# mnlevy1981/MOM6

Measured on AMD Instinct MI355X. Metric: simulated-years/day (SYPD) of the split-RK2 dynamical core + tracer advection + ALE remap, higher is better.
Workload: dtype f64

## Files before the change

### include/mom6hip.h

```cpp
#ifndef MOM6HIP_H
#define MOM6HIP_H

#include <stdint.h>

#ifdef __cplusplus
extern "C" {
#endif

#define MOM6HIP_MEM_HOST   0
#define MOM6HIP_MEM_DEVICE 1

#define MOM6HIP_ADV_PLM    0
#define MOM6HIP_ADV_PPM_H3 1
#define MOM6HIP_ADV_PPM    2

typedef struct mom6hip_grid {
  int32_t isc, iec, jsc, jec;
  int32_t isd, ied, jsd, jed;
  int32_t nk;
  int32_t symmetric;
  int32_t reentrant_x, reentrant_y;
  int32_t first_direction;
  int32_t tripolar_n;
  double Angstrom_H;
// ... 331 lines not shown
                           const mom6hip_bt_cont_t *BT_cont, double *du_cor, double *dv_cor, int32_t memspace);


#define MOM6HIP_EOS_LINEAR 1
#define MOM6HIP_EOS_UNESCO 2
#define MOM6HIP_EOS_WRIGHT 3
#define MOM6HIP_EOS_WRIGHT_FULL 4
#define MOM6HIP_EOS_WRIGHT_REDUCED 5

typedef struct mom6hip_eos {
  int32_t form;
  int32_t reserved;
  double Rho_T0_S0, dRho_dT, dRho_dS;
} mom6hip_eos_t;

typedef struct mom6hip_pressureforce_cs {
  double Rho0;
  double GFS_scale;
  double Z_ref;
  int32_t reconstruct;
  int32_t Recon_Scheme;
  int32_t boundary_extrap;
  int32_t useMassWghtInterp;
  int32_t use_ALE;
  int32_t nkmb;
  double P_Ref;
  const double *Rlay;
  const double *g_prime;
} mom6hip_pressureforce_cs_t;

int mom6hip_pressureforce_fv_bouss(mom6hip_ctx_t *ctx, const mom6hip_pressureforce_cs_t *cs, const mom6hip_eos_t *eos,
                                   const double *h, const double *T, const double *S, const double *p_atm,
                                   double *PFu, double *PFv, double *pbce, double *eta, int32_t memspace);

int mom6hip_pressureforce_fv_nonbouss(mom6hip_ctx_t *ctx, const mom6hip_pressureforce_cs_t *cs, const mom6hip_eos_t *eos,
                                      const double *h, const double *T, const double *S, const double *p_atm, double H_to_RZ,
                                      double *PFu, double *PFv, double *pbce, double *eta, int32_t memspace);

int mom6hip_calculate_density(mom6hip_ctx_t *ctx, const mom6hip_eos_t *eos, const double *T, const double *S,
                              const double *pressure, double *rho, int64_t n, int32_t use_rho_ref, double rho_ref,
                              int32_t memspace);


#define MOM6HIP_BT_HARMONIC     1
#define MOM6HIP_BT_ARITHMETIC   2
#define MOM6HIP_BT_HYBRID       3
#define MOM6HIP_BT_FROM_BT_CONT 4

typedef struct mom6hip_barotropic_cs {
  double dtbt;
  double dtbt_max;
  double dtbt_fraction;
  double bebt;
  double dt_bt_filter;
  double vel_underflow;
  double G_extra;
  double BT_Coriolis_scale;
  double Z_ref;
  double maxCFL_BT_cont;
  double reserved0[6];
  int32_t Sadourny;
  int32_t linearized_BT_PV;
  int32_t strong_drag;
  int32_t visc_rem_u_uh0;
  int32_t adjust_BT_cont;
  int32_t use_wide_halos;
// ... 416 lines not shown
```

### mom6_amd/_lib.py

```python
import ctypes as C
import os

from . import _abi

_HERE = os.path.dirname(os.path.abspath(__file__))
LIB_PATH = os.environ.get("MOM6HIP_LIB_PATH") or os.path.join(_HERE, "libmom6hip.so")
_LIB = None
_dp = C.POINTER(C.c_double)

EXPORTS = (
    "mom6hip_init", "mom6hip_last_error", "mom6hip_grid_create", "mom6hip_grid_destroy",
    "mom6hip_sync", "mom6hip_malloc", "mom6hip_free", "mom6hip_sync_to_device",
    "mom6hip_sync_to_host", "mom6hip_halo_update", "mom6hip_advect_tracer", "mom6hip_set_timing",
    "mom6hip_advect_get_timing", "mom6hip_ale_remap_tracers", "mom6hip_ale_plm_edge_values", "mom6hip_coradcalc", "mom6hip_continuity", "mom6hip_pressureforce_fv_bouss", "mom6hip_pressureforce_fv_nonbouss", "mom6hip_calculate_density", "mom6hip_set_domain_callbacks",
    "mom6hip_barotropic_init", "mom6hip_btcalc", "mom6hip_bt_mass_source", "mom6hip_set_dtbt", "mom6hip_memset_zero", "mom6hip_transfer_stats", "mom6hip_debug_poison_passes", "mom6hip_tracer_hordiff_varmix", "mom6hip_tracer_hordiff_neutral", "mom6hip_tracer_hordiff_epipycnal", "mom6hip_continuity_obc", "mom6hip_coradcalc_obc", "mom6hip_vertvisc_coef_obc", "mom6hip_update_segment_tracer_reservoirs", "mom6hip_advect_tracer_obc", "mom6hip_btstep_obc", "mom6hip_horizontal_viscosity_obc", "mom6hip_set_viscous_bbl_obc", "mom6hip_btcalc_obc", "mom6hip_vertvisc_obc", "mom6hip_radiation_open_bdry_conds", "mom6hip_open_boundary_zero_normal_flow", "mom6hip_overlap_stats", "mom6hip_thickness_diffuse", "mom6hip_mixedlayer_restrat", "mom6hip_mixedlayer_restrat_mu", "mom6hip_start_group_pass", "mom6hip_complete_group_pass", "mom6hip_set_dtbt_eta", "mom6hip_btstep",
    "mom6hip_dyn_split_rk2_init", "mom6hip_step_dyn_split_rk2", "mom6hip_dyn_split_rk2b_init", "mom6hip_step_dyn_split_rk2b",
    "mom6hip_ale_regrid", "mom6hip_ale_remap_set_h_vel", "mom6hip_ale_remap_set_h_vel_via_dz", "mom6hip_ale_remap_velocities", "mom6hip_halo_pack", "mom6hip_set_min_callback", "mom6hip_kernel_timing", "mom6hip_set_callback_stream_ordered", "mom6hip_bt_graph_stats", "mom6hip_bt_graph_nodes",
    "mom6hip_vertvisc_coef", "mom6hip_vertvisc", "mom6hip_vertvisc_remnant", "mom6hip_vertvisc_ntrunc", "mom6hip_vertvisc_and_remnant", "mom6hip_vertvisc_step",
    "mom6hip_hor_visc_init", "mom6hip_horizontal_viscosity", "mom6hip_set_viscous_bbl", "mom6hip_set_viscous_ml",
    "mom6hip_chksum", "mom6hip_reproducing_sum", "mom6hip_write_energy_sums", "mom6hip_depth_list_create", "mom6hip_write_energy_ape", "mom6hip_host_register", "mom6hip_host_unregister", "mom6hip_stage_to_host",
    "mom6hip_stage_query", "mom6hip_stage_wait", "mom6hip_stream_bandwidth", "mom6hip_graph_node_floor", "mom6hip_tracer_hordiff", "mom6hip_tracer_hordiff_hbd", "mom6hip_rccl_get_unique_id", "mom6hip_domain_init_rccl", "mom6hip_domain_exchange_timing",
)


class Mom6HipError(RuntimeError):
    pass


def lib():
    global _LIB
    if _LIB is None:
        if not os.path.exists(LIB_PATH):
            raise Mom6HipError(
                f"{LIB_PATH} not found: build it with `python -c 'import __graft_entry__ as g; g.build()'` "
                "(make -C mom6_amd/csrc). mom6_amd has no CPU fallback.")
        import importlib.util
        if importlib.util.find_spec("torch") is not None:
            import torch
        L = C.CDLL(LIB_PATH)
        L.mom6hip_last_error.restype = C.c_char_p
        L.mom6hip_init.argtypes = [C.c_int]
        L.mom6hip_grid_create.argtypes = [C.POINTER(_abi.GridStruct), C.c_void_p, C.POINTER(C.c_void_p)]
        L.mom6hip_grid_destroy.argtypes = [C.c_void_p]
        L.mom6hip_sync.argtypes = [C.c_void_p]
        L.mom6hip_malloc.argtypes = [C.POINTER(C.c_void_p), C.c_uint64]
        L.mom6hip_free.argtypes = [C.c_void_p]
        L.mom6hip_sync_to_device.argtypes = [C.c_void_p, C.c_void_p, C.c_void_p, C.c_uint64]
# ... 41 lines not shown
```

### mom6_amd/csrc/common.hpp

```cpp
#pragma once

#include <hip/hip_runtime.h>
#include <cstdint>
#include <cstdio>
#include <cstring>
#include <functional>
#include <string>
#include <utility>
#include <vector>

#include "../../include/mom6hip.h"

struct mom6hip_ctx;
struct m6_native_domain;

namespace m6 {

void set_error(const char *fmt, ...);
struct ErrorKeeper {
  ErrorKeeper();
  ~ErrorKeeper();
  char saved[1024];
};

// ... 42 lines not shown
struct DevBuf {
  void *p = nullptr;
  size_t bytes = 0;
  int reserve(size_t n);
  void release();
};

struct HostTable {
  DevBuf buf;
  std::vector<double> last;
  const double *get(const double *host, size_t n);
};
enum { TABLE_PGF_RLAY = 0, TABLE_PGF_GPRIME, TABLE_SVML_RLAY, TABLE_TD_RLAY, TABLE_TD_GPRIME, TABLE_COUNT = 8 };

}

struct mom6hip_ctx {
  mom6hip_grid_t host;
  m6::GridDev g;
  hipStream_t stream = nullptr;
  std::vector<void *> metric_allocs;
  double *d_metric[64] = {};

  m6::DevBuf hprev, uhr, vhr, flags, stage[16], tr_stage[64];
  m6::DevBuf pool[64];
  m6::DevBuf rk2_scratch;
  m6::DevBuf rk2_eta_PF_start;
  int rk2_scratch_layout = 0;
  m6::DevBuf hv_pack;
  bool hv_pack_ready = false;
  m6::DevBuf hv_str;
  m6::DevBuf cont_hmid;
  uint64_t overlap[4] = {0, 0, 0, 0};
  int cont_phase = 0;
  struct BcAccelFuse { const double *au, *av, *diffu, *diffv; double *u_bc, *v_bc; int inviscid; bool done; };
  BcAccelFuse *bc_fuse = nullptr;
  bool cont_fluxes_only = false;
  m6::DevBuf sv_rlay;
  m6::DevBuf adv_gen;
  m6::DevBuf adv_obc[64];
  int adv_obc_n = 0;
  m6::HostTable tables[m6::TABLE_COUNT];
  uint64_t xfer[4] = {0, 0, 0, 0};
  m6::DevBuf ale_sub;
  m6::DevBuf ale_side;
  std::vector<const void *> lds_configured;
  struct ObcTable { int site; uint64_t key; m6::DevBuf buf; size_t bytes; uint64_t last_use; std::vector<char> host; };
  std::vector<ObcTable> obc_tables;
  uint64_t obc_table_clock = 0, obc_table_builds = 0;
  m6::DevBuf vv_ntrunc;
  bool vv_ntrunc_ready = false;
  std::vector<std::pair<std::string, void *>> bt_graphs;
  hipStream_t cap_stream = nullptr;
  static constexpr int NSIDE = 4;
  hipStream_t side_stream[NSIDE] = {nullptr, nullptr, nullptr, nullptr};
  hipEvent_t side_fork = nullptr, side_join[NSIDE] = {nullptr, nullptr, nullptr, nullptr};
  long bt_graph_captures = 0, bt_graph_launches = 0, bt_graph_nodes_last = 0;
  int *h_domore_k = nullptr;
  m6_native_domain *native = nullptr;
  mom6hip_halo_fn halo_cb = nullptr;
  mom6hip_sum_fn sum_cb = nullptr;
  bool cb_stream_ordered = false;
  mom6hip_min_fn min_cb = nullptr;
  void *min_user = nullptr;
  void *cb_user = nullptr;
  int num_PEs = 0;
// ... 109 lines not shown
```

### mom6_amd/csrc/eos.hpp

```cpp
#pragma once

#include "common.hpp"

namespace m6 {
namespace eos {

struct EosDev { int form; double Rho_T0_S0, dRho_dT, dRho_dS; };

constexpr double a0 = 7.057924e-4, a1 = 3.480336e-7, a2 = -1.112733e-7;
constexpr double b0 = 5.790749e8, b1 = 3.516535e6, b2 = -4.002714e4, b3 = 2.084372e2, b4 = 5.944068e5, b5 = -9.643486e3;
constexpr double c0 = 1.704853e5, c1 = 7.904722e2, c2 = -7.984422, c3 = 5.140652e-2, c4 = -2.302158e2, c5 = -3.079464;

namespace unesco {
constexpr double R00 = 999.842594, R01 = 6.793952e-2, R02 = -9.095290e-3, R03 = 1.001685e-4, R04 = -1.120083e-6, R05 = 6.536332e-9,
    R10 = 0.824493, R11 = -4.0899e-3, R12 = 7.6438e-5, R13 = -8.2467e-7, R14 = 5.3875e-9, R60 = -5.72466e-3, R61 = 1.0227e-4,
    R62 = -1.6546e-6, R20 = 4.8314e-4,
    S000 = 1.965933e4, S010 = 1.444304e2, S020 = -1.706103, S030 = 9.648704e-3, S040 = -4.190253e-5, S100 = 52.84855,
    S110 = -3.101089e-1, S120 = 6.283263e-3, S130 = -5.084188e-5, S600 = 3.886640e-1, S610 = 9.085835e-3, S620 = -4.619924e-4,
    S001 = 3.186519, S011 = 2.212276e-2, S021 = -2.984642e-4, S031 = 1.956415e-6, S101 = 6.704388e-3, S111 = -1.847318e-4,
    S121 = 2.059331e-7, S601 = 1.480266e-4,
    S002 = 2.102898e-4, S012 = -1.202016e-5, S022 = 1.394680e-7, S102 = -2.040237e-6, S112 = 6.128773e-8, S122 = 6.207323e-10;
__device__ __forceinline__ double density(double T, double S, double pressure) {
  const double p1 = pressure*1.0e-5, t1 = T;
  const double s1 = (S > 0.0 ? S : 0.0), s12 = sqrt(s1);
// ... 69 lines not shown
  const double lam_TS = W.c4*S + T * (W.c1 + (T*(W.c2 + W.c3*T) + W.c5*S));
  return (pa_000 + (p_TSp - rho_ref*(p_TSp*al0 + (W.b0*al_TS + lam_TS)))) / ( (W.c0 + lam_TS) + al0*(W.b0 + p_TSp) );
}
__device__ __forceinline__ double wrightx_spv_anomaly(const WrightCoefs W, double T, double S, double pressure, double spv_ref) {
  const double lam_000 = W.c0 + (W.a0 - spv_ref)*W.b0;
  const double al_TS = W.a1*T + W.a2*S;
  const double p_TSp = pressure + (W.b4*S + T * (W.b1 + (T*(W.b2 + W.b3*T) + W.b5*S)));
  const double lambda = lam_000 + ( W.c4*S + T * (W.c1 + (T*(W.c2 + W.c3*T) + W.c5*S)) );
  return al_TS + (lambda + (W.a0 - spv_ref)*p_TSp) / (W.b0 + p_TSp);
}
__device__ __forceinline__ void wrightx_density_derivs(const WrightCoefs W, double T, double S, double pressure, double &DT, double &DS) {
  const double al0 = W.a0 + (W.a1*T + W.a2*S);
  const double p0 = W.b0 + ( W.b4*S + T * (W.b1 + (T*(W.b2 + W.b3*T) + W.b5*S)) );
  const double lambda = W.c0 + ( W.c4*S + T * (W.c1 + (T*(W.c2 + W.c3*T) + W.c5*S)) );
  const double den = (lambda + al0*(pressure + p0));
  const double I_denom2 = 1.0 / (den*den);
  DT = I_denom2 * (lambda * (W.b1 + (T*(2.0*W.b2 + 3.0*W.b3*T) + W.b5*S)) -
     (pressure+p0) * ( (pressure+p0)*W.a1 + (W.c1 + (T*(W.c2*2.0 + W.c3*3.0*T) + W.c5*S)) ));
  DS = I_denom2 * (lambda * (W.b4 + W.b5*T) -
     (pressure+p0) * ( (pressure+p0)*W.a2 + (W.c4 + W.c5*T) ));
}
__device__ __forceinline__ bool is_wrightx(int form) { return form == MOM6HIP_EOS_WRIGHT_FULL || form == MOM6HIP_EOS_WRIGHT_REDUCED; }

__device__ __forceinline__ double eos_density(const EosDev &E, double T, double S, double pressure) {
  if (E.form == MOM6HIP_EOS_LINEAR) return E.Rho_T0_S0 + E.dRho_dT * T + E.dRho_dS * S;
  if (E.form == MOM6HIP_EOS_UNESCO) return unesco::density(T, S, pressure);
  if (is_wrightx(E.form)) return wrightx_density(wright_coefs(E.form), T, S, pressure);
  const double al0 = (a0 + a1 * T) + a2 * S;
  const double p0 = (b0 + b4 * S) + T * (b1 + T * (b2 + b3 * T) + b5 * S);
  const double lambda = (c0 + c4 * S) + T * (c1 + T * (c2 + c3 * T) + c5 * S);
  return (pressure + p0) / (lambda + al0 * (pressure + p0));
}

__device__ __forceinline__ double eos_density_anomaly(const EosDev &E, double T, double S, double pressure, double rho_ref) {
  if (E.form == MOM6HIP_EOS_LINEAR) return (E.Rho_T0_S0 - rho_ref) + (E.dRho_dT * T + E.dRho_dS * S);
  if (E.form == MOM6HIP_EOS_UNESCO) return unesco::density_anomaly(T, S, pressure, rho_ref);
  if (is_wrightx(E.form)) return wrightx_density_anomaly(wright_coefs(E.form), T, S, pressure, rho_ref);
  const double pa_000 = (b0 * (1.0 - a0 * rho_ref) - rho_ref * c0);
  const double al_TS = a1 * T + a2 * S;
  const double al0 = a0 + al_TS;
  const double p_TSp = pressure + (b4 * S + T * (b1 + (T * (b2 + b3 * T) + b5 * S)));
  const double lam_TS = c4 * S + T * (c1 + (T * (c2 + c3 * T) + c5 * S));
  return (pa_000 + (p_TSp - rho_ref * (p_TSp * al0 + (b0 * al_TS + lam_TS)))) / ((c0 + lam_TS) + al0 * (b0 + p_TSp));
}

__device__ __forceinline__ void eos_density_derivs(const EosDev &E, double T, double S, double pressure, double &drho_dT,
                                                   double &drho_dS) {
  if (E.form == MOM6HIP_EOS_LINEAR) { drho_dT = E.dRho_dT; drho_dS = E.dRho_dS; return; }
  if (E.form == MOM6HIP_EOS_UNESCO) { unesco::density_derivs(T, S, pressure, drho_dT, drho_dS); return; }
  if (is_wrightx(E.form)) { wrightx_density_derivs(wright_coefs(E.form), T, S, pressure, drho_dT, drho_dS); return; }
  const double al0 = (a0 + a1 * T) + a2 * S;
  const double p0 = (b0 + b4 * S) + T * (b1 + T * ((b2 + b3 * T)) + b5 * S);
  const double lambda = (c0 + c4 * S) + T * (c1 + T * ((c2 + c3 * T)) + c5 * S);
  double I_denom2 = 1.0 / (lambda + al0 * (pressure + p0));
  I_denom2 = I_denom2 * I_denom2;
  drho_dT = I_denom2 * (lambda * (b1 + T * (2.0 * b2 + 3.0 * b3 * T) + b5 * S) -
                        (pressure + p0) * ((pressure + p0) * a1 + (c1 + T * (c2 * 2.0 + c3 * 3.0 * T) + c5 * S)));
  drho_dS = I_denom2 * (lambda * (b4 + b5 * T) - (pressure + p0) * ((pressure + p0) * a2 + (c4 + c5 * T)));
}

__device__ __forceinline__ double eos_spec_vol_anomaly(const EosDev &E, double T, double S, double pressure, double spv_ref) {
  if (E.form == MOM6HIP_EOS_LINEAR)
    return ((1.0 - E.Rho_T0_S0*spv_ref) - spv_ref*(E.dRho_dT*T + E.dRho_dS*S)) / (E.Rho_T0_S0 + (E.dRho_dT*T + E.dRho_dS*S));
  if (is_wrightx(E.form)) return wrightx_spv_anomaly(wright_coefs(E.form), T, S, pressure, spv_ref);
  if (E.form == MOM6HIP_EOS_UNESCO) {
    using namespace unesco;
    const double p1 = pressure*1.0e-5, t1 = T;
    const double s1 = (S > 0.0 ? S : 0.0), s12 = sqrt(s1);
    const double rho0 = R00 + ( t1*(R01 + t1*(R02 + t1*(R03 + t1*(R04 + t1*R05)))) +
                   s1*((R10 + t1*(R11 + t1*(R12 + t1*(R13 + t1*R14)))) +
// ... 17 lines not shown
```

### mom6_amd/csrc/pressure_force.hip

```cpp
#include <cmath>

#include "common.hpp"
#include "eos.hpp"

namespace {

using m6::max2;
using m6::min2;
using namespace m6::eos;
__device__ __forceinline__ double max3(double a, double b, double c) { return max2(max2(a, b), c); }
__device__ __forceinline__ double min3(double a, double b, double c) { return min2(min2(a, b), c); }
__device__ __forceinline__ double fsign(double a, double b) { return copysign(fabs(a), b); }

__device__ double plm_slope_wa(double h_l, double h_c, double h_r, double h_neglect, double u_l, double u_c, double u_r) {
  const double sigma_r = u_r - u_c;
  const double sigma_l = u_c - u_l;
  const double sigma_c = 2.0 * (u_r - u_l) * (h_c / (h_l + 2.0 * h_c + h_r + h_neglect));
  const double u_min = min3(u_l, u_c, u_r);
  const double u_max = max3(u_l, u_c, u_r);
  double slope = 0.0;
  if ((sigma_l * sigma_r) > 0.0) slope = fsign(min2(fabs(sigma_c), 2. * min2(u_c - u_min, u_max - u_c)), sigma_c);
  if (u_c - 0.5 * fabs(slope) < u_min || u_c + 0.5 * fabs(slope) > u_max) slope = slope * (1. - 2.220446049250313e-16);
  if (fabs(slope) < 1.E-140) slope = 0.;
  return slope;
// ... 113 lines not shown
    const double iz = 0.5 * G_e * (dz * dz) * (rho_anom - C1_90 * (16.0 * (r5[3] - r5[1]) + 7.0 * (r5[4] - r5[0])));
    p.intz_dpa[o3] = iz * g.Z_to_H;

    if (p.pbce) {
      const double press = -Rho0xG * (e_K - p.Z_ref);
      double pb;
      if (kk == 0) {
        const double rho_in_situ = eos_density(p.eos, T_c, S_c, press);
        pb = G_Rho0 * (p.GFS_scale * rho_in_situ) * g.H_to_Z;
      } else {
        const double T_int = 0.5 * (T_m + T_c), S_int = 0.5 * (S_m + S_c);
        double dR_dT, dR_dS;
        eos_density_derivs(p.eos, T_int, S_int, press, dR_dT, dR_dS);
        pb = pbce_prev + G_Rho0 * ((e_K - e_bot) * Ihtot) * (dR_dT * (T_c - T_m) + dR_dS * (S_c - S_m));
      }
      p.pbce[o3] = pb;
      pbce_prev = pb;
    }

    e_K = e_Kp1;
    h_m = h_c; h_c = h_p; h_p = h_q; h_q = ld(p.h, kk + 3);
    T_m = T_c; T_c = T_p; T_p = T_q; T_q = ld(p.T, kk + 3);
    S_m = S_c; S_c = S_p; S_p = S_q; S_q = ld(p.S, kk + 3);
    sT_m = sT_c; sT_c = sT_p; sS_m = sS_c; sS_c = sS_p;
    if (kk + 2 <= nz - 2) {
      sT_p = plm_slope_wa(h_c, h_p, h_q, h_neglect, T_c, T_p, T_q);
      sS_p = plm_slope_wa(h_c, h_p, h_q, h_neglect, S_c, S_p, S_q);
    } else {
      sT_p = 0.; sS_p = 0.;
    }
  }
}

__device__ __forceinline__ double face_integral(const PgfArgs &p, long oL3, long oR3, long oL2, long oR2, double eL_K,
                                                double eL_Kp1, double eR_K, double eR_Kp1) {
  const m6::GridDev &g = p.g;
  const double G_e = g.g_Earth, GxRho = G_e * p.rho_ref, rho_ref = p.rho_ref;
  const double C1_90 = 1.0 / 90.0;
  double Ttl, Tbl, Ttr, Tbr, Stl, Sbl, Str, Sbr;
  const double TtL = p.T_t[oL3], TtR = p.T_t[oR3], TbL = p.T_b[oL3], TbR = p.T_b[oR3];
  const double StL = p.S_t[oL3], StR = p.S_t[oR3], SbL = p.S_b[oL3], SbR = p.S_b[oR3];
  double hWght = (p.massw ? 1. : 0.) * max3(0., -g.bathyT[oL2] - eR_K, -g.bathyT[oR2] - eL_K);
  if (hWght > 0.) {
    const double hL = (eL_K - eL_Kp1) + g.dZ_subroundoff;
    const double hR = (eR_K - eR_Kp1) + g.dZ_subroundoff;
    const double rr = (hL - hR) / (hL + hR);
    hWght = hWght * (rr * rr);
    const double iDenom = 1. / (hWght * (hR + hL) + hL * hR);
    Ttl = ((hWght * hR) * TtR + (hWght * hL + hR * hL) * TtL) * iDenom;
    Ttr = ((hWght * hL) * TtL + (hWght * hR + hR * hL) * TtR) * iDenom;
    Tbl = ((hWght * hR) * TbR + (hWght * hL + hR * hL) * TbL) * iDenom;
    Tbr = ((hWght * hL) * TbL + (hWght * hR + hR * hL) * TbR) * iDenom;
    Stl = ((hWght * hR) * StR + (hWght * hL + hR * hL) * StL) * iDenom;
    Str = ((hWght * hL) * StL + (hWght * hR + hR * hL) * StR) * iDenom;
    Sbl = ((hWght * hR) * SbR + (hWght * hL + hR * hL) * SbL) * iDenom;
    Sbr = ((hWght * hL) * SbL + (hWght * hR + hR * hL) * SbR) * iDenom;
  } else {
    Ttl = TtL; Tbl = TbL; Ttr = TtR; Tbr = TbR;
    Stl = StL; Sbl = SbL; Str = StR; Sbr = SbR;
  }
  double intz[5];
  intz[0] = p.dpa[oL3]; intz[4] = p.dpa[oR3];
#pragma unroll
  for (int m = 2; m <= 4; m++) {
    const double w_left = 0.25 * (double)(5 - m), w_right = 1.0 - w_left;
    const double dz_x = w_left * (eL_K - eL_Kp1) + w_right * (eR_K - eR_Kp1);
    const double T1 = w_left * Ttl + w_right * Ttr, T5 = w_left * Tbl + w_right * Tbr;
    const double S1 = w_left * Stl + w_right * Str, S5 = w_left * Sbl + w_right * Sbr;
    double pn = -GxRho * ((w_left * eL_K + w_right * eR_K) - p.Z_ref);
    double r[5];
#pragma unroll
    for (int n = 1; n <= 5; n++) {
      if (n > 1) pn = pn + GxRho * 0.25 * dz_x;
      double Tn, Sn;
      if (n == 1) { Tn = T1; Sn = S1; }
      else if (n == 5) { Tn = T5; Sn = S5; }
      else {
        const double wt_t = 0.25 * (double)(5 - n), wt_b = 1.0 - wt_t;
        Sn = wt_t * S1 + wt_b * S5;
        Tn = wt_t * T1 + wt_b * T5;
      }
      r[n - 1] = eos_density_anomaly(p.eos, Tn, Sn, pn, rho_ref);
    }
    intz[m - 1] = G_e * dz_x * (C1_90 * (7.0 * (r[0] + r[4]) + 32.0 * (r[1] + r[3]) + 12.0 * r[2]));
  }
  return C1_90 * (7.0 * (intz[0] + intz[4]) + 32.0 * (intz[1] + intz[3]) + 12.0 * intz[2]);
}

__global__ __launch_bounds__(64, PGF_FACE_OCC) void pgf_face_kernel(PgfArgs p) {
  const m6::GridDev &g = p.g;
  const int i = g.isc - 1 + blockIdx.x * 64 + threadIdx.x;
  const int j = g.jsc - 1 + blockIdx.y;
  if (i > g.iec) return;
  const bool do_x = (j >= g.jsc), do_y = (i >= g.isc);
  if (!do_x && !do_y) return;
  const int nz = g.nk;
  const long pl = (long)g.nih * g.njh, plU = (long)(g.nih + 1) * g.njh, plV = (long)g.nih * (g.njh + 1);
  const long oc = g.h2(i, j), oe = oc + 1, on = oc + g.nih;
  const double h_neglect = g.H_subroundoff, I_Rho0 = 1.0 / g.Rho0;
  const double rg = p.rho_ref * g.g_Earth;
  auto pa0 = [&](long o2) -> double {
    double v = rg * (p.e[o2] - p.Z_ref);
    if (p.p_atm) v = v + p.p_atm[o2];
    return v;
  };
  double pa_c = pa0(oc), pa_e = do_x ? pa0(oe) : 0.0, pa_n = do_y ? pa0(on) : 0.0;
  double intx_pa = 0.5 * (pa_c + pa_e), inty_pa = 0.5 * (pa_c + pa_n);
  const double fx = do_x ? (2.0 * I_Rho0 * g.IdxCu[g.u2(i, j)]) : 0.0;
  const double fy = do_y ? (2.0 * I_Rho0 * g.IdyCv[g.v2(i, j)]) : 0.0;
  double ec_K = p.e[oc], ee_K = do_x ? p.e[oe] : 0.0, en_K = do_y ? p.e[on] : 0.0;
  for (int k = 0; k < nz; k++) {
    const long c3 = oc + pl * k;
    const double ec_Kp1 = p.e[c3 + pl];
    const double h_c = p.h[c3], dpa_c = p.dpa[c3], iz_c = p.intz_dpa[c3];
    if (do_x) {
      const long e3 = c3 + 1;
      const double ee_Kp1 = p.e[e3 + pl];
      const double h_e = p.h[e3];
      const double intx_dpa = face_integral(p, c3, e3, oc, oe, ec_K, ec_Kp1, ee_K, ee_Kp1);
// ... 5 lines not shown
        const long n = g.u2(i, j) + plU * k;
        double a = p.bc_CAu[n] + pfu;
        if (p.bc_inviscid) a = (a == 0.0) ? 0.0 : a; else a = a + p.bc_diffu[n];
        p.bc_u[n] = a;
      }
      intx_pa = intx_pa + intx_dpa;
      pa_e = pa_e + p.dpa[e3];
      ee_K = ee_Kp1;
    }
    if (do_y) {
      const long n3 = c3 + g.nih;
      const double en_Kp1 = p.e[n3 + pl];
      const double h_n = p.h[n3];
      const double inty_dpa = face_integral(p, c3, n3, oc, on, ec_K, ec_Kp1, en_K, en_Kp1);
      const double pfv = (((pa_c * h_c + iz_c) - (pa_n * h_n + p.intz_dpa[n3])) +
                          ((h_n - h_c) * inty_pa - (en_Kp1 - ec_Kp1) * inty_dpa * g.Z_to_H)) *
                         (fy / ((h_c + h_n) + h_neglect));
      p.PFv[g.v2(i, j) + plV * k] = pfv;
      if (p.bc_v) {
        const long n = g.v2(i, j) + plV * k;
        double a = p.bc_CAv[n] + pfv;
        if (p.bc_inviscid) a = (a == 0.0) ? 0.0 : a; else a = a + p.bc_diffv[n];
        p.bc_v[n] = a;
      }
      inty_pa = inty_pa + inty_dpa;
      pa_n = pa_n + p.dpa[n3];
      en_K = en_Kp1;
    }
    pa_c = pa_c + dpa_c;
    ec_K = ec_Kp1;
  }
}

struct PlmEdgeArgs { m6::GridDev g; const double *h, *Q; double *Q_t, *Q_b; int bdry_extrap; };
__global__ __launch_bounds__(64) void plm_edge_kernel(PlmEdgeArgs p) {
  const m6::GridDev &g = p.g;
  const int i = g.isc - 1 + blockIdx.x * 64 + threadIdx.x;
  const int j = g.jsc - 1 + blockIdx.y;
  if (i > g.iec + 1) return;
  const int nz = g.nk;
  const long o2 = g.h2(i, j), pl = (long)g.nih * g.njh;
  const double h_neglect = g.H_subroundoff;
  auto ld = [&](const double *a, int kk) -> double { return (kk >= 0 && kk < nz) ? a[o2 + pl * kk] : 0.0; };
  double h_m = 0., h_c = ld(p.h, 0), h_p = ld(p.h, 1), h_q = ld(p.h, 2);
  double Q_m = 0., Q_c = ld(p.Q, 0), Q_p = ld(p.Q, 1), Q_q = ld(p.Q, 2);
  double s_m = 0., s_c = 0., s_p = 0.;
  if (nz >= 3) s_p = plm_slope_wa(h_c, h_p, h_q, h_neglect, Q_c, Q_p, Q_q);
  for (int kk = 0; kk < nz; kk++) {
    double Qt, Qb;
    if (kk >= 1 && kk <= nz - 2) {
      const double m = plm_monotonized_slope(Q_m, Q_c, Q_p, s_m, s_c, s_p);
      Qt = Q_c - 0.5 * m; Qb = Q_c + 0.5 * m;
    } else if (p.bdry_extrap) {
      const double m = kk == 0 ? -plm_extrapolate_slope(h_p, h_c, h_neglect, Q_p, Q_c) : plm_extrapolate_slope(h_m, h_c, h_neglect, Q_m, Q_c);
      Qt = Q_c - 0.5 * m; Qb = Q_c + 0.5 * m;
    } else {
      Qt = Q_c; Qb = Q_c;
    }
    p.Q_t[o2 + pl * kk] = Qt; p.Q_b[o2 + pl * kk] = Qb;
    h_m = h_c; h_c = h_p; h_p = h_q; h_q = ld(p.h, kk + 3);
    Q_m = Q_c; Q_c = Q_p; Q_p = Q_q; Q_q = ld(p.Q, kk + 3);
    s_m = s_c; s_c = s_p;
    s_p = (kk + 2 <= nz - 2) ? plm_slope_wa(h_c, h_p, h_q, h_neglect, Q_c, Q_p, Q_q) : 0.;
  }
}

// ... 520 lines not shown
    a.Rlay = ctx->tables[m6::TABLE_PGF_RLAY].get(cs->Rlay, (size_t)g.nk);
    if (!a.Rlay) return 1;
  }
  if (mode == PCM_NOEOS && pbce) {
    a.g_prime = ctx->tables[m6::TABLE_PGF_GPRIME].get(cs->g_prime, (size_t)g.nk + 1);
    if (!a.g_prime) return 1;
  }
  m6::Stager st(ctx, memspace);
  a.g = g;
  a.eos = use_EOS ? EosDev{eos->form, eos->Rho_T0_S0, eos->dRho_dT, eos->dRho_dS} : EosDev{0, 0., 0., 0.};
  a.h = st.in(h, bH); a.T = use_EOS ? st.in(T, bH) : nullptr; a.S = use_EOS ? st.in(S, bH) : nullptr; a.p_atm = st.in(p_atm, bH2);
  a.PFu = st.inout(PFu, bU); a.PFv = st.inout(PFv, bV); a.pbce = st.inout(pbce, bH); a.eta = st.inout(eta, bH2);
  a.e = (double *)st.scratch(bH + bH2);
  a.T_t = a.T_b = a.S_t = a.S_b = nullptr;
  if (use_ALE) {
    a.T_t = (double *)st.scratch(bH); a.T_b = (double *)st.scratch(bH);
    a.S_t = (double *)st.scratch(bH); a.S_b = (double *)st.scratch(bH);
  }
  a.dpa = (double *)st.scratch(bH); a.intz_dpa = (double *)st.scratch(bH);
  if (st.failed()) return 1;
  a.rho_ref = cs->Rho0; a.Z_ref = cs->Z_ref; a.GFS_scale = cs->GFS_scale; a.za0 = nullptr; a.H_to_RZ = 0.0;
  a.boundary_extrap = cs->boundary_extrap; a.massw = cs->useMassWghtInterp;
  a.nkmb = use_EOS ? cs->nkmb : 0; a.P_Ref = cs->P_Ref;
  const int ncol_i = g.iec - g.isc + 3, ncol_j = g.jec - g.jsc + 3;
  const dim3 gc((ncol_i + 63) / 64, ncol_j), gf((ncol_i - 1 + 63) / 64, ncol_j - 1);
  if (use_ALE) {
    if (ctx->bc_fuse && memspace == MOM6HIP_MEM_DEVICE) {
      mom6hip_ctx::BcAccelFuse *f = ctx->bc_fuse;
      a.bc_CAu = f->au; a.bc_CAv = f->av; a.bc_diffu = f->diffu; a.bc_diffv = f->diffv; a.bc_u = f->u_bc; a.bc_v = f->v_bc;
      a.bc_inviscid = f->inviscid;
      f->done = true;
    }
    hipLaunchKernelGGL(pgf_column_kernel, gc, dim3(64), 0, s, a);
    { m6::KTimer kt(ctx, MOM6HIP_KT_PGF_FACE); hipLaunchKernelGGL(pgf_face_kernel, gf, dim3(64), 0, s, a); }
  } else if (mode == PCM_LINEAR) {
    hipLaunchKernelGGL(pgf_pcm_column_kernel<PCM_LINEAR>, gc, dim3(64), 0, s, a);
    hipLaunchKernelGGL(pgf_pcm_face_kernel<PCM_LINEAR>, gf, dim3(64), 0, s, a);
  } else if (mode == PCM_WRIGHT) {
    hipLaunchKernelGGL(pgf_pcm_column_kernel<PCM_WRIGHT>, gc, dim3(64), 0, s, a);
    hipLaunchKernelGGL(pgf_pcm_face_kernel<PCM_WRIGHT>, gf, dim3(64), 0, s, a);
  } else {
    hipLaunchKernelGGL(pgf_pcm_column_kernel<PCM_NOEOS>, gc, dim3(64), 0, s, a);
    hipLaunchKernelGGL(pgf_pcm_face_kernel<PCM_NOEOS>, gf, dim3(64), 0, s, a);
  }
  M6_HIP(hipGetLastError());
  return st.finish();
}

extern "C" int mom6hip_pressureforce_fv_nonbouss(mom6hip_ctx_t *ctx, const mom6hip_pressureforce_cs_t *cs,
                                                 const mom6hip_eos_t *eos, const double *h, const double *T,
                                                 const double *S, const double *p_atm, double H_to_RZ, double *PFu,
                                                 double *PFv, double *pbce, double *eta, int32_t memspace) {
  M6_REQUIRE(ctx != nullptr && cs != nullptr, "MOM_PressureForce_FV_nonBouss: Module must be initialized before it is used.");
  M6_REQUIRE(h && T && S && PFu && PFv, "PressureForce_FV_nonBouss: null argument");
  M6_REQUIRE(memspace == MOM6HIP_MEM_HOST || memspace == MOM6HIP_MEM_DEVICE, "PressureForce_FV_nonBouss: bad memspace");
  if (check_eos(eos)) return 2;
  M6_REQUIRE(cs->use_ALE && cs->reconstruct && cs->Recon_Scheme == 1,
             "PressureForce_FV_nonBouss: only ALE with RECONSTRUCT_FOR_PRESSURE=True and PRESSURE_RECONSTRUCTION_SCHEME=1 is provided");
  M6_REQUIRE(cs->GFS_scale == 1.0, "PressureForce_FV_nonBouss: GFS_scale < 1 is not provided");
  M6_REQUIRE(H_to_RZ > 0.0, "PressureForce_FV_nonBouss: H_to_RZ must be positive");
  m6::GridDev &g = ctx->g;
  M6_REQUIRE(g.bathyT && g.IdxCu && g.IdyCv, "PressureForce_FV_nonBouss: a required grid metric is missing");
  M6_REQUIRE(g.nk >= 2, "PressureForce_FV_nonBouss: at least 2 layers are needed");
  M6_REQUIRE(g.isc - g.isd >= 1 && g.ied - g.iec >= 1 && g.jsc - g.jsd >= 1 && g.jed - g.jec >= 1,
             "PressureForce_FV_nonBouss: needs a halo of at least 1");
  hipStream_t s = ctx->stream;
  const size_t bH = (size_t)g.nh3() * 8, bU = (size_t)g.nu3() * 8, bV = (size_t)g.nv3() * 8;
  const size_t bH2 = (size_t)g.nih * g.njh * 8;
  m6::Stager st(ctx, memspace);
  PgfArgs a;
  a.bc_CAu = a.bc_CAv = a.bc_diffu = a.bc_diffv = nullptr; a.bc_u = a.bc_v = nullptr; a.bc_inviscid = 0;
  a.g = g;
  a.eos = EosDev{eos->form, eos->Rho_T0_S0, eos->dRho_dT, eos->dRho_dS};
  a.h = st.in(h, bH); a.T = st.in(T, bH); a.S = st.in(S, bH); a.p_atm = st.in(p_atm, bH2);
  a.PFu = st.inout(PFu, bU); a.PFv = st.inout(PFv, bV); a.pbce = st.inout(pbce, bH); a.eta = st.inout(eta, bH2);
  a.e = (double *)st.scratch(bH + bH2);
  a.T_t = (double *)st.scratch(bH); a.T_b = (double *)st.scratch(bH);
  a.S_t = (double *)st.scratch(bH); a.S_b = (double *)st.scratch(bH);
  a.dpa = (double *)st.scratch(bH); a.intz_dpa = (double *)st.scratch(bH);
// ... 31 lines not shown
```

### mom6_amd/pressure_force.py

```python
from __future__ import annotations

import ctypes as C

from . import _abi
from ._lib import Mom6HipError, check, lib
from .tracer_advect import DeviceGrid, _ptr_space


def EOS_init(form="WRIGHT", Rho_T0_S0=1000.0, dRho_dT=-0.2, dRho_dS=0.8):
    if form not in _abi.EOS_FORMS:
        raise Mom6HipError("interpret_eos_selection: EQN_OF_STATE " + str(form) + " is not provided by libmom6hip "
                           "(WRIGHT, WRIGHT_FULL, WRIGHT_REDUCED, UNESCO, LINEAR)")
    return _abi.EOS(_abi.EOS_FORMS[form], 0, float(Rho_T0_S0), float(dRho_dT), float(dRho_dS))


def calculate_density(T, S, pressure, rho, EOS, G: DeviceGrid, rho_ref=None):
    spaces = set()
    n = None
    ptrs = []
    for a in (T, S, pressure, rho):
        p, sp = _ptr_space(a)
        spaces.add(sp); ptrs.append(C.c_void_p(p))
        m = int(a.numel()) if hasattr(a, "numel") else int(a.size)
        if n is not None and m != n:
            raise Mom6HipError("calculate_density: T, S, pressure and rho must have the same number of points")
        n = m
    if len(spaces) != 1:
        raise Mom6HipError("calculate_density: all fields must be in the same memory space")
    L = lib()
    L.mom6hip_calculate_density.argtypes = ([C.c_void_p, C.POINTER(_abi.EOS)] + [C.c_void_p] * 4 + [C.c_int64, C.c_int32, C.c_double, C.c_int32])
    check(L.mom6hip_calculate_density(G.handle, C.byref(EOS), *ptrs, n, 0 if rho_ref is None else 1, 0.0 if rho_ref is None else float(rho_ref),
                                      spaces.pop()), "calculate_density")


def PressureForce_init(grid, Rho0=None, boundary_extrap=True, useMassWghtInterp=False, Z_ref=0.0, reconstruct=True, use_ALE=True,
                       nk_rho_varies=0, P_Ref=2.0e7, Rlay=None, g_prime=None):
    import numpy as np
    cs = _abi.PressureForceCS(float(grid.Rho0 if Rho0 is None else Rho0), 1.0, float(Z_ref), int(bool(reconstruct)), 1,
                              int(bool(boundary_extrap)), int(bool(useMassWghtInterp)), int(bool(use_ALE)), int(nk_rho_varies),
                              float(P_Ref), None, None)
    cs._keep = []
    for name, a in (("Rlay", Rlay), ("g_prime", g_prime)):
        if a is not None:
            a = np.ascontiguousarray(a, dtype=np.float64); cs._keep.append(a)
            setattr(cs, name, a.ctypes.data)
    return cs


def PressureForce(h, tv, PFu, PFv, G: DeviceGrid, CS, ALE_CSp=None, p_atm=None, pbce=None, eta=None, Boussinesq=True, H_to_RZ=1.0):
    if CS is None:
        raise Mom6HipError("MOM_PressureForce_FV_Bouss: Module must be initialized before it is used.")
    T, S, EOS = tv
    spaces = set()

    def P(a):
        if a is None:
            return None
        p, s = _ptr_space(a)
        spaces.add(s)
        return C.c_void_p(p)

    args = [P(x) for x in (h, T, S, p_atm, PFu, PFv, pbce, eta)]
    if len(spaces) != 1:
        raise Mom6HipError("PressureForce: all fields must be in the same memory space")
    if not Boussinesq:
# ... 6 lines not shown
```

Baseline: 25.40.

## Add templated pressure-gradient face kernel specialized on EOS, mass weighting and BC

Adds a templated variant of the pressure-gradient face kernel that fixes the equation-of-state form (Wright only), mass-weighted interpolation, boundary-condition fusion mode and atmospheric pressure presence at compile time. It also uses 32-bit byte offsets for addressing and can optionally prefetch the next layer's column data. The aim is to remove runtime branching, shrink register use and address arithmetic, and let the compiler schedule the quadrature EOS evaluations better. The cost is more kernel instantiations, plus a fallback to the generic kernel for other EOS forms or very large grids. A launch counter is added to show which path runs.

```diff
diff --git a/include/mom6hip.h b/include/mom6hip.h
--- a/include/mom6hip.h
+++ b/include/mom6hip.h
@@ -387,6 +387,7 @@
 int mom6hip_pressureforce_fv_bouss(mom6hip_ctx_t *ctx, const mom6hip_pressureforce_cs_t *cs, const mom6hip_eos_t *eos,
                                    const double *h, const double *T, const double *S, const double *p_atm,
                                    double *PFu, double *PFv, double *pbce, double *eta, int32_t memspace);
+int mom6hip_pgf_face_launches(mom6hip_ctx_t *ctx, uint64_t *counts);
 
 int mom6hip_pressureforce_fv_nonbouss(mom6hip_ctx_t *ctx, const mom6hip_pressureforce_cs_t *cs, const mom6hip_eos_t *eos,
                                       const double *h, const double *T, const double *S, const double *p_atm, double H_to_RZ,
diff --git a/mom6_amd/_lib.py b/mom6_amd/_lib.py
--- a/mom6_amd/_lib.py
+++ b/mom6_amd/_lib.py
@@ -12,7 +12,7 @@
     "mom6hip_init", "mom6hip_last_error", "mom6hip_grid_create", "mom6hip_grid_destroy",
     "mom6hip_sync", "mom6hip_malloc", "mom6hip_free", "mom6hip_sync_to_device",
     "mom6hip_sync_to_host", "mom6hip_halo_update", "mom6hip_advect_tracer", "mom6hip_set_timing",
-    "mom6hip_advect_get_timing", "mom6hip_ale_remap_tracers", "mom6hip_ale_plm_edge_values", "mom6hip_coradcalc", "mom6hip_continuity", "mom6hip_pressureforce_fv_bouss", "mom6hip_pressureforce_fv_nonbouss", "mom6hip_calculate_density", "mom6hip_set_domain_callbacks",
+    "mom6hip_advect_get_timing", "mom6hip_ale_remap_tracers", "mom6hip_ale_plm_edge_values", "mom6hip_coradcalc", "mom6hip_continuity", "mom6hip_pressureforce_fv_bouss", "mom6hip_pressureforce_fv_nonbouss", "mom6hip_pgf_face_launches", "mom6hip_calculate_density", "mom6hip_set_domain_callbacks",
     "mom6hip_barotropic_init", "mom6hip_btcalc", "mom6hip_bt_mass_source", "mom6hip_set_dtbt", "mom6hip_memset_zero", "mom6hip_transfer_stats", "mom6hip_debug_poison_passes", "mom6hip_tracer_hordiff_varmix", "mom6hip_tracer_hordiff_neutral", "mom6hip_tracer_hordiff_epipycnal", "mom6hip_continuity_obc", "mom6hip_coradcalc_obc", "mom6hip_vertvisc_coef_obc", "mom6hip_update_segment_tracer_reservoirs", "mom6hip_advect_tracer_obc", "mom6hip_btstep_obc", "mom6hip_horizontal_viscosity_obc", "mom6hip_set_viscous_bbl_obc", "mom6hip_btcalc_obc", "mom6hip_vertvisc_obc", "mom6hip_radiation_open_bdry_conds", "mom6hip_open_boundary_zero_normal_flow", "mom6hip_overlap_stats", "mom6hip_thickness_diffuse", "mom6hip_mixedlayer_restrat", "mom6hip_mixedlayer_restrat_mu", "mom6hip_start_group_pass", "mom6hip_complete_group_pass", "mom6hip_set_dtbt_eta", "mom6hip_btstep",
     "mom6hip_dyn_split_rk2_init", "mom6hip_step_dyn_split_rk2", "mom6hip_dyn_split_rk2b_init", "mom6hip_step_dyn_split_rk2b",
     "mom6hip_ale_regrid", "mom6hip_ale_remap_set_h_vel", "mom6hip_ale_remap_set_h_vel_via_dz", "mom6hip_ale_remap_velocities", "mom6hip_halo_pack", "mom6hip_set_min_callback", "mom6hip_kernel_timing", "mom6hip_set_callback_stream_ordered", "mom6hip_bt_graph_stats", "mom6hip_bt_graph_nodes",
diff --git a/mom6_amd/csrc/common.hpp b/mom6_amd/csrc/common.hpp
--- a/mom6_amd/csrc/common.hpp
+++ b/mom6_amd/csrc/common.hpp
@@ -98,6 +98,7 @@
   m6::DevBuf hv_str;
   m6::DevBuf cont_hmid;
   uint64_t overlap[4] = {0, 0, 0, 0};
+  uint64_t pgf_face_launches[2] = {0, 0};
   int cont_phase = 0;
   struct BcAccelFuse { const double *au, *av, *diffu, *diffv; double *u_bc, *v_bc; int inviscid; bool done; };
   BcAccelFuse *bc_fuse = nullptr;
diff --git a/mom6_amd/csrc/eos.hpp b/mom6_amd/csrc/eos.hpp
--- a/mom6_amd/csrc/eos.hpp
+++ b/mom6_amd/csrc/eos.hpp
@@ -125,10 +125,13 @@
   return (pressure + p0) / (lambda + al0 * (pressure + p0));
 }
 
+constexpr int EOS_FORM_RUNTIME = -1;
+template <int FORM = EOS_FORM_RUNTIME>
 __device__ __forceinline__ double eos_density_anomaly(const EosDev &E, double T, double S, double pressure, double rho_ref) {
-  if (E.form == MOM6HIP_EOS_LINEAR) return (E.Rho_T0_S0 - rho_ref) + (E.dRho_dT * T + E.dRho_dS * S);
-  if (E.form == MOM6HIP_EOS_UNESCO) return unesco::density_anomaly(T, S, pressure, rho_ref);
-  if (is_wrightx(E.form)) return wrightx_density_anomaly(wright_coefs(E.form), T, S, pressure, rho_ref);
+  const int form = (FORM == EOS_FORM_RUNTIME) ? E.form : FORM;
+  if (form == MOM6HIP_EOS_LINEAR) return (E.Rho_T0_S0 - rho_ref) + (E.dRho_dT * T + E.dRho_dS * S);
+  if (form == MOM6HIP_EOS_UNESCO) return unesco::density_anomaly(T, S, pressure, rho_ref);
+  if (is_wrightx(form)) return wrightx_density_anomaly(wright_coefs(form), T, S, pressure, rho_ref);
   const double pa_000 = (b0 * (1.0 - a0 * rho_ref) - rho_ref * c0);
   const double al_TS = a1 * T + a2 * S;
   const double al0 = a0 + al_TS;
diff --git a/mom6_amd/csrc/pressure_force.hip b/mom6_amd/csrc/pressure_force.hip
--- a/mom6_amd/csrc/pressure_force.hip
+++ b/mom6_amd/csrc/pressure_force.hip
@@ -169,15 +169,22 @@
   }
 }
 
-__device__ __forceinline__ double face_integral(const PgfArgs &p, long oL3, long oR3, long oL2, long oR2, double eL_K,
-                                                double eL_Kp1, double eR_K, double eR_Kp1) {
+struct PgfColK { double e_Kp1, Tt, Tb, St, Sb, dpa; };
+constexpr int PGF_RUNTIME = -1;
+
+template <int FORM, int MASSW, bool FENCE = false>
+__device__ __forceinline__ double face_integral_core(const PgfArgs &p, const PgfColK &L, const PgfColK &R, double bathyL, double bathyR,
+                                                     double eL_K, double eR_K) {
   const m6::GridDev &g = p.g;
   const double G_e = g.g_Earth, GxRho = G_e * p.rho_ref, rho_ref = p.rho_ref;
   const double C1_90 = 1.0 / 90.0;
+  const double eL_Kp1 = L.e_Kp1, eR_Kp1 = R.e_Kp1;
   double Ttl, Tbl, Ttr, Tbr, Stl, Sbl, Str, Sbr;
-  const double TtL = p.T_t[oL3], TtR = p.T_t[oR3], TbL = p.T_b[oL3], TbR = p.T_b[oR3];
-  const double StL = p.S_t[oL3], StR = p.S_t[oR3], SbL = p.S_b[oL3], SbR = p.S_b[oR3];
-  double hWght = (p.massw ? 1. : 0.) * max3(0., -g.bathyT[oL2] - eR_K, -g.bathyT[oR2] - eL_K);
+  const double TtL = L.Tt, TtR = R.Tt, TbL = L.Tb, TbR = R.Tb;
+  const double StL = L.St, StR = R.St, SbL = L.Sb, SbR = R.Sb;
+  const bool massw = (MASSW == PGF_RUNTIME) ? (p.massw != 0) : (MASSW != 0);
+  double hWght = 0.;
+  if (MASSW != 0) hWght = (massw ? 1. : 0.) * max3(0., -bathyL - eR_K, -bathyR - eL_K);
   if (hWght > 0.) {
     const double hL = (eL_K - eL_Kp1) + g.dZ_subroundoff;
     const double hR = (eR_K - eR_Kp1) + g.dZ_subroundoff;
@@ -197,7 +204,7 @@
     Stl = StL; Sbl = SbL; Str = StR; Sbr = SbR;
   }
   double intz[5];
-  intz[0] = p.dpa[oL3]; intz[4] = p.dpa[oR3];
+  intz[0] = L.dpa; intz[4] = R.dpa;
 #pragma unroll
   for (int m = 2; m <= 4; m++) {
     const double w_left = 0.25 * (double)(5 - m), w_right = 1.0 - w_left;
@@ -217,11 +224,22 @@
         Sn = wt_t * S1 + wt_b * S5;
         Tn = wt_t * T1 + wt_b * T5;
       }
-      r[n - 1] = eos_density_anomaly(p.eos, Tn, Sn, pn, rho_ref);
+      r[n - 1] = eos_density_anomaly<FORM>(p.eos, Tn, Sn, pn, rho_ref);
     }
     intz[m - 1] = G_e * dz_x * (C1_90 * (7.0 * (r[0] + r[4]) + 32.0 * (r[1] + r[3]) + 12.0 * r[2]));
+    if (FENCE) __builtin_amdgcn_sched_barrier(0);
   }
   return C1_90 * (7.0 * (intz[0] + intz[4]) + 32.0 * (intz[1] + intz[3]) + 12.0 * intz[2]);
+}
+
+__device__ __forceinline__ double face_integral(const PgfArgs &p, long oL3, long oR3, long oL2, long oR2, double eL_K,
+                                                double eL_Kp1, double eR_K, double eR_Kp1) {
+  PgfColK L, R;
+  L.e_Kp1 = eL_Kp1; R.e_Kp1 = eR_Kp1;
+  L.Tt = p.T_t[oL3]; R.Tt = p.T_t[oR3]; L.Tb = p.T_b[oL3]; R.Tb = p.T_b[oR3];
+  L.St = p.S_t[oL3]; R.St = p.S_t[oR3]; L.Sb = p.S_b[oL3]; R.Sb = p.S_b[oR3];
+  L.dpa = p.dpa[oL3]; R.dpa = p.dpa[oR3];
+  return face_integral_core<EOS_FORM_RUNTIME, PGF_RUNTIME>(p, L, R, p.g.bathyT[oL2], p.g.bathyT[oR2], eL_K, eR_K);
 }
 
 __global__ __launch_bounds__(64, PGF_FACE_OCC) void pgf_face_kernel(PgfArgs p) {
@@ -293,6 +311,158 @@
   }
 }
 
+#ifndef PGF_FACE_T_OCC
+#define PGF_FACE_T_OCC 3
+#endif
+#ifndef PGF_FACE_PF
+#define PGF_FACE_PF 0
+#endif
+#ifndef PGF_FACE_FENCE
+#define PGF_FACE_FENCE 0
+#endif
+constexpr int PGF_BC_OFF = 0, PGF_BC_VISCOUS = 1, PGF_BC_INVISCID = 2;
+struct PgfColLate { double h, iz; };
+__device__ __forceinline__ double pgf_ld(const double *a, unsigned b) { return *(const double *)((const char *)a + b); }
+__device__ __forceinline__ void pgf_st(double *a, unsigned b, double v) { *(double *)((char *)a + b) = v; }
+__device__ __forceinline__ PgfColK pgf_load_col(const PgfArgs &p, unsigned b, unsigned plb) {
+  PgfColK c;
+  c.e_Kp1 = pgf_ld(p.e, b + plb); c.Tt = pgf_ld(p.T_t, b); c.Tb = pgf_ld(p.T_b, b); c.St = pgf_ld(p.S_t, b); c.Sb = pgf_ld(p.S_b, b);
+  c.dpa = pgf_ld(p.dpa, b);
+  return c;
+}
+__device__ __forceinline__ PgfColLate pgf_load_late(const PgfArgs &p, unsigned b) {
+  PgfColLate c;
+  c.h = pgf_ld(p.h, b); c.iz = pgf_ld(p.intz_dpa, b);
+  return c;
+}
+
+template <int FORM, bool MASSW, int BC, bool PATM>
+__global__ __launch_bounds__(64, PGF_FACE_T_OCC) void pgf_face_kernel_t(PgfArgs p) {
+  const m6::GridDev &g = p.g;
+  const int i = g.isc - 1 + blockIdx.x * 64 + threadIdx.x;
+  const int j = g.jsc - 1 + blockIdx.y;
+  if (i > g.iec) return;
+  const bool do_x = (j >= g.jsc), do_y = (i >= g.isc);
+  if (!do_x && !do_y) return;
+  const int nz = g.nk;
+  const long oc = g.h2(i, j), oe = do_x ? oc + 1 : oc, on = do_y ? oc + g.nih : oc;
+  const long ou = g.u2(i, j), ov = g.v2(i, j);
+  const unsigned pl = 8u * (unsigned)(g.nih * g.njh), plU = 8u * (unsigned)((g.nih + 1) * g.njh), plV = 8u * (unsigned)(g.nih * (g.njh + 1));
+  unsigned c3 = 8u * (unsigned)oc, e3 = 8u * (unsigned)oe, n3 = 8u * (unsigned)on, u3 = 8u * (unsigned)ou, v3 = 8u * (unsigned)ov;
+  const double h_neglect = g.H_subroundoff, I_Rho0 = 1.0 / g.Rho0;
+  const double rg = p.rho_ref * g.g_Earth;
+  auto pa0 = [&](long o2) -> double {
+    double v = rg * (p.e[o2] - p.Z_ref);
+    if (PATM) v = v + p.p_atm[o2];
+    return v;
+  };
+  double pa_c = pa0(oc), pa_e = pa0(oe), pa_n = pa0(on);
+  double intx_pa = 0.5 * (pa_c + pa_e), inty_pa = 0.5 * (pa_c + pa_n);
+  const double fx = do_x ? (2.0 * I_Rho0 * g.IdxCu[ou]) : 0.0;
+  const double fy = do_y ? (2.0 * I_Rho0 * g.IdyCv[ov]) : 0.0;
+  double bathy_c = 0., bathy_e = 0., bathy_n = 0.;
+  if (MASSW) { bathy_c = g.bathyT[oc]; bathy_e = g.bathyT[oe]; bathy_n = g.bathyT[on]; }
+  double ec_K = p.e[oc], ee_K = p.e[oe], en_K = p.e[on];
+#if PGF_FACE_PF >= 1
+  PgfColK c = pgf_load_col(p, c3, pl), e = pgf_load_col(p, e3, pl), n = pgf_load_col(p, n3, pl);
+#endif
+#if PGF_FACE_PF == 2
+  PgfColLate lc = pgf_load_late(p, c3), le = pgf_load_late(p, e3), ln = pgf_load_late(p, n3);
+  double cau = 0., cav = 0., dfu = 0., dfv = 0.;
+  if (BC != PGF_BC_OFF) { cau = pgf_ld(p.bc_CAu, u3); cav = pgf_ld(p.bc_CAv, v3); }
+  if (BC == PGF_BC_VISCOUS) { dfu = pgf_ld(p.bc_diffu, u3); dfv = pgf_ld(p.bc_diffv, v3); }
+#endif
+  for (int k = 0; k < nz; k++) {
+    const unsigned dn = (k + 1 < nz) ? pl : 0u, dnU = (k + 1 < nz) ? plU : 0u, dnV = (k + 1 < nz) ? plV : 0u;
+    (void)dn; (void)dnU; (void)dnV;
+#if PGF_FACE_PF >= 1
+    const PgfColK c1 = pgf_load_col(p, c3 + dn, pl), e1 = pgf_load_col(p, e3 + dn, pl), n1 = pgf_load_col(p, n3 + dn, pl);
+#else
+    const PgfColK c = pgf_load_col(p, c3, pl), e = pgf_load_col(p, e3, pl), n = pgf_load_col(p, n3, pl);
+#endif
+#if PGF_FACE_PF == 2
+    const PgfColLate lc1 = pgf_load_late(p, c3 + dn), le1 = pgf_load_late(p, e3 + dn), ln1 = pgf_load_late(p, n3 + dn);
+    double cau1 = 0., cav1 = 0., dfu1 = 0., dfv1 = 0.;
+    if (BC != PGF_BC_OFF) { cau1 = pgf_ld(p.bc_CAu, u3 + dnU); cav1 = pgf_ld(p.bc_CAv, v3 + dnV); }
+    if (BC == PGF_BC_VISCOUS) { dfu1 = pgf_ld(p.bc_diffu, u3 + dnU); dfv1 = pgf_ld(p.bc_diffv, v3 + dnV); }
+#else
+    const PgfColLate lc = pgf_load_late(p, c3), le = pgf_load_late(p, e3), ln = pgf_load_late(p, n3);
+    double cau = 0., cav = 0., dfu = 0., dfv = 0.;
+    if (BC != PGF_BC_OFF) { cau = pgf_ld(p.bc_CAu, u3); cav = pgf_ld(p.bc_CAv, v3); }
+    if (BC == PGF_BC_VISCOUS) { dfu = pgf_ld(p.bc_diffu, u3); dfv = pgf_ld(p.bc_diffv, v3); }
+#endif
+    const double intx_dpa = face_integral_core<FORM, MASSW ? 1 : 0, PGF_FACE_FENCE == 2>(p, c, e, bathy_c, bathy_e, ec_K, ee_K);
+#if PGF_FACE_FENCE
+    __builtin_amdgcn_sched_barrier(0);
+#endif
+    const double inty_dpa = face_integral_core<FORM, MASSW ? 1 : 0, PGF_FACE_FENCE == 2>(p, c, n, bathy_c, bathy_n, ec_K, en_K);
+#if PGF_FACE_FENCE
+    __builtin_amdgcn_sched_barrier(0);
+#endif
+    const double h_c = lc.h, iz_c = lc.iz, ec_Kp1 = c.e_Kp1;
+    {
+      const double ee_Kp1 = e.e_Kp1, h_e = le.h;
+      const double pfu = (((pa_c * h_c + iz_c) - (pa_e * h_e + le.iz)) +
+                          ((h_e - h_c) * intx_pa - (ee_Kp1 - ec_Kp1) * intx_dpa * g.Z_to_H)) *
+                         (fx / ((h_c + h_e) + h_neglect));
+      if (do_x) {
+        pgf_st(p.PFu, u3, pfu);
+        if (BC != PGF_BC_OFF) {
+          double a = cau + pfu;
+          if (BC == PGF_BC_INVISCID) a = (a == 0.0) ? 0.0 : a; else a = a + dfu;
+          pgf_st(p.bc_u, u3, a);
+        }
+      }
+      intx_pa = intx_pa + intx_dpa;
+      pa_e = pa_e + e.dpa;
+      ee_K = ee_Kp1;
+    }
+    {
+      const double en_Kp1 = n.e_Kp1, h_n = ln.h;
+      const double pfv = (((pa_c * h_c + iz_c) - (pa_n * h_n + ln.iz)) +
+                          ((h_n - h_c) * inty_pa - (en_Kp1 - ec_Kp1) * inty_dpa * g.Z_to_H)) *
+                         (fy / ((h_c + h_n) + h_neglect));
+      if (do_y) {
+        pgf_st(p.PFv, v3, pfv);
+        if (BC != PGF_BC_OFF) {
+          double a = cav + pfv;
+          if (BC == PGF_BC_INVISCID) a = (a == 0.0) ? 0.0 : a; else a = a + dfv;
+          pgf_st(p.bc_v, v3, a);
+        }
+      }
+      inty_pa = inty_pa + inty_dpa;
+      pa_n = pa_n + n.dpa;
+      en_K = en_Kp1;
+    }
+    pa_c = pa_c + c.dpa;
+    ec_K = ec_Kp1;
+    c3 += pl; e3 += pl; n3 += pl; u3 += plU; v3 += plV;
+#if PGF_FACE_PF >= 1
+    c = c1; e = e1; n = n1;
+#endif
+#if PGF_FACE_PF == 2
+    lc = lc1; le = le1; ln = ln1; cau = cau1; cav = cav1; dfu = dfu1; dfv = dfv1;
+#endif
+  }
+}
+
+using PgfFaceKernel = void (*)(PgfArgs);
+template <int FORM>
+PgfFaceKernel pgf_face_pick_form(bool massw, int bc, bool patm) {
+#define PGF_T(M, B) (patm ? pgf_face_kernel_t<FORM, M, B, true> : pgf_face_kernel_t<FORM, M, B, false>)
+  if (massw) return bc == PGF_BC_OFF ? PGF_T(true, PGF_BC_OFF) : bc == PGF_BC_VISCOUS ? PGF_T(true, PGF_BC_VISCOUS) : PGF_T(true, PGF_BC_INVISCID);
+  return bc == PGF_BC_OFF ? PGF_T(false, PGF_BC_OFF) : bc == PGF_BC_VISCOUS ? PGF_T(false, PGF_BC_VISCOUS) : PGF_T(false, PGF_BC_INVISCID);
+#undef PGF_T
+}
+PgfFaceKernel pgf_face_pick(const PgfArgs &a) {
+  const uint64_t planes = (uint64_t)a.g.nk + 1, pmax = (uint64_t)(a.g.nih + 1) * (uint64_t)(a.g.njh + 1);
+  if (planes * pmax * 8 >= (1ull << 32)) return nullptr;
+  if (!a.bc_u != !a.bc_v) return nullptr;
+  const int bc = !a.bc_u ? PGF_BC_OFF : a.bc_inviscid ? PGF_BC_INVISCID : PGF_BC_VISCOUS;
+  if (a.eos.form == MOM6HIP_EOS_WRIGHT) return pgf_face_pick_form<MOM6HIP_EOS_WRIGHT>(a.massw != 0, bc, a.p_atm != nullptr);
+  return nullptr;
+}
+
 struct PlmEdgeArgs { m6::GridDev g; const double *h, *Q; double *Q_t, *Q_b; int bdry_extrap; };
 __global__ __launch_bounds__(64) void plm_edge_kernel(PlmEdgeArgs p) {
   const m6::GridDev &g = p.g;
@@ -879,7 +1049,9 @@
       f->done = true;
     }
     hipLaunchKernelGGL(pgf_column_kernel, gc, dim3(64), 0, s, a);
-    { m6::KTimer kt(ctx, MOM6HIP_KT_PGF_FACE); hipLaunchKernelGGL(pgf_face_kernel, gf, dim3(64), 0, s, a); }
+    const PgfFaceKernel face_t = pgf_face_pick(a);
+    ctx->pgf_face_launches[face_t ? 1 : 0]++;
+    { m6::KTimer kt(ctx, MOM6HIP_KT_PGF_FACE); hipLaunchKernelGGL(face_t ? face_t : pgf_face_kernel, gf, dim3(64), 0, s, a); }
   } else if (mode == PCM_LINEAR) {
     hipLaunchKernelGGL(pgf_pcm_column_kernel<PCM_LINEAR>, gc, dim3(64), 0, s, a);
     hipLaunchKernelGGL(pgf_pcm_face_kernel<PCM_LINEAR>, gf, dim3(64), 0, s, a);
@@ -892,6 +1064,12 @@
   }
   M6_HIP(hipGetLastError());
   return st.finish();
+}
+
+extern "C" int mom6hip_pgf_face_launches(mom6hip_ctx_t *ctx, uint64_t *counts) {
+  M6_REQUIRE(ctx != nullptr && counts != nullptr, "mom6hip_pgf_face_launches: null argument");
+  counts[0] = ctx->pgf_face_launches[0]; counts[1] = ctx->pgf_face_launches[1];
+  return 0;
 }
 
 extern "C" int mom6hip_pressureforce_fv_nonbouss(mom6hip_ctx_t *ctx, const mom6hip_pressureforce_cs_t *cs,
diff --git a/mom6_amd/pressure_force.py b/mom6_amd/pressure_force.py
--- a/mom6_amd/pressure_force.py
+++ b/mom6_amd/pressure_force.py
@@ -31,6 +31,13 @@
     L.mom6hip_calculate_density.argtypes = ([C.c_void_p, C.POINTER(_abi.EOS)] + [C.c_void_p] * 4 + [C.c_int64, C.c_int32, C.c_double, C.c_int32])
     check(L.mom6hip_calculate_density(G.handle, C.byref(EOS), *ptrs, n, 0 if rho_ref is None else 1, 0.0 if rho_ref is None else float(rho_ref),
                                       spaces.pop()), "calculate_density")
+
+
+def pgf_face_launches(G: DeviceGrid):
+    L = lib(); L.mom6hip_pgf_face_launches.argtypes = [C.c_void_p, C.POINTER(C.c_uint64)]
+    out = (C.c_uint64 * 2)()
+    check(L.mom6hip_pgf_face_launches(G.handle, out), "mom6hip_pgf_face_launches")
+    return int(out[0]), int(out[1])
 
 
 def PressureForce_init(grid, Rho0=None, boundary_extrap=True, useMassWghtInterp=False, Z_ref=0.0, reconstruct=True, use_ALE=True,
```

Measured after the change: 25.92, median of 6. 1.02x the previous value.
